# dayoladejo/GADMM

Measured on AMD Instinct MI355X. Metric: wall-clock to 1e-8 objective gap, GADMM linear regression (LinearRegression_Synthetic), lower is better.
Workload: dtype fp64; 1 GPU; model=LinearRegression_Synthetic GADMM closed-form, workers=24, features=50, samples_per_worker=50, global_batch=1200, seq_len=1, parallelism=chain24-over-1gpu

## Files before the change

### csrc/kernels/chain_blocked.hip

```cpp
#include "gadmm_common.h"
#include "gadmm_chain.h"
#include "persist_device.h"
#include "persist_launch.h"
#include <stdlib.h>

namespace {

constexpr int MAXW = 12;
constexpr int HIMG52 = 4 * 64 * 14;
constexpr int EPL = 256;
constexpr long DYN_LDS_BYTES = (long)MAXW * EPL * (16 + 8 + 4);
struct EpochLds {
  int4* sl;
  int2* fl;
  int* st;
};
__device__ __forceinline__ EpochLds epoch_lds(double* base, int v) {
  int4* sl = reinterpret_cast<int4*>(base);
  int2* fl = reinterpret_cast<int2*>(sl + MAXW * EPL);
  int* st = reinterpret_cast<int*>(fl + MAXW * EPL);
  return {sl + v * EPL, fl + v * EPL, st + v * EPL};
}

template <int QT>
__device__ __forceinline__ void quad_load_image(double (&m)[4][QT], const double* img) {
  const int lane = threadIdx.x & 63;
  const double2* p = reinterpret_cast<const double2*>(img) + lane;
#pragma unroll
  for (int t = 0; t < QT; t += 2)
#pragma unroll
    for (int r = 0; r < 4; ++r) {
      const double2 v = p[((t >> 1) * 4 + r) * 64];
      m[r][t] = v.x;
      if (t + 1 < QT) m[r][t + 1] = v.y;
    }
}

template <class PA>
__device__ __forceinline__ void stage_epochs(const PA& a, int q, const EpochLds& el, bool flush) {
  const int lane = threadIdx.x & 63;
  for (int e = lane; e < a.n_epochs; e += 64) {
    el.sl[e] = reinterpret_cast<const int4*>(a.ep_slots)[(long)e * a.n + q];
    if (flush) el.fl[e] = reinterpret_cast<const int2*>(a.ep_flush)[(long)e * a.n + q];
    el.st[e] = a.epoch_start[e];
  }
}
}



template <int QT, bool SYS, bool DYN = false, class PA = PersistArgs>
__device__ __forceinline__ void blocked_objective(const PA& a, double* lds, int v, int lane, int q,
                                                  unsigned long long deadline, __amdgpu_buffer_rsrc_t rob,
                                                  __amdgpu_buffer_rsrc_t rtab, bool local = false) {
  const int d = a.d, n = a.n;
  const long ring_base = 2L * n * 2 * d;
  const EpochLds el = epoch_lds(lds + MAXW * 64 + MAXW * QSTAGE, v);
  int* posl = reinterpret_cast<int*>(el.fl);
  if constexpr (DYN) {
    for (int e = lane; e < a.n_epochs; e += 64) {
      posl[e] = a.ep_pos[(long)e * n + q];
      el.st[e] = a.epoch_start[e];
    }
  }
  const PhaseSlot so = a.slots[DYN ? 0 : q];
  const int li = DYN ? q : so.li, gid = DYN ? q : so.gid;
  int row = DYN ? posl[0] : q;
  const bool in = lane < d;
  double Aq[4][QT];
  quad_load<QT>(Aq, a.A + (long)li * d * d, d, true);
  const double bo = in ? a.b[(long)li * d + lane] : 0.0;
  const double hy = 0.5 * a.yy[li];
  double* xo = lds + v * QSTAGE;
  int ep = 0, next_start = (DYN && a.n_epochs > 1) ? el.st[1] : 0x7fffffff;
  for (int it = a.start_iter;; ++it) {
    if (a.hard_stop > 0 && it > a.hard_stop) return;
    if constexpr (DYN) {
      if (it == next_start) {
        ++ep;
        next_start = ep + 1 < a.n_epochs ? el.st[ep + 1] : 0x7fffffff;
        row = posl[ep];
      }
    }
    const unsigned tag = make_tag(a.epoch, it);
    const long off = (ring_base + ((long)(it % a.ring) * n + row) * d + lane) * 16;
    double x = 0.0;
    for (int spin = 0;; ++spin) {
      const bool ok = !in || load_granule<SYS>(rtab, (int)off, tag, &x);
      if (__all(ok)) break;
      if ((spin & 7) == 7) {
        if (it - a.start_iter >= a.lag) {
          const unsigned long long dv = load_dec<SYS>(&a.decg[(it - a.lag) % a.ring]);
          if ((unsigned)(dv >> 32) == make_tag(a.epoch, it - a.lag) && (unsigned)(dv & 0xffffffffu) != 0u) return;
        }
        if (now_ticks() > deadline) return;
      }
      GADMM_POLL_PAUSE();
    }
    const double qv = quad_gemv<QT>(Aq, in ? x : 0.0, xo);
    const double part = in ? (0.5 * qv - bo) * x : 0.0;
    const double f = wave_sum_f64(part) + hy;
    if (lane == 0) put_granule<SYS>(local, rob, ((it % a.ring) * n + gid) * 16, tag, f);
  }
}

template <int DB, bool SYS, bool TL, bool DYN, bool HALO, bool SWEEP, class PA>
__device__ __forceinline__ void chain_blocked_body(const PA& a) {
  constexpr int QT = DB / 4;
  extern __shared__ __attribute__((aligned(16))) double lds[];
  __shared__ int abort_lds, stop_lds, stop_iter_lds;
  const int d = a.d, n = a.n;
  const int lane = threadIdx.x & 63;
  const int v = __builtin_amdgcn_readfirstlane(threadIdx.x >> 6);
  const int k = a.blk_k, L = a.blk_len, H = 2 * a.blk_k;
  const bool multi = a.nranks > 1;
  const int seg_lo = multi ? a.seg_lo : 0, seg_hi = multi ? a.seg_hi : n - 1;
  const int nseg = seg_hi - seg_lo + 1;
  const int W = (nseg + L - 1) / L;
  const int Wo = (nseg + MAXW - 1) / MAXW;
  const bool dl = SYS && multi && a.blk_dl != 0;
  const unsigned long long deadline = now_ticks() + (unsigned long long)a.timeout_ticks;
  const __amdgpu_buffer_rsrc_t rob = rsrc_of(a.objg);
  const __amdgpu_buffer_rsrc_t rtab = rsrc_of(a.blk_tab);
  const bool packed = SWEEP || (!SYS && a.xcd > 0);
  if (!SWEEP && packed && (blockIdx.x & 7u)) return;
  const int bid = packed ? (int)(blockIdx.x >> 3) : (int)blockIdx.x;
  if (SWEEP && bid > W + Wo) return;
  if (threadIdx.x == 0) {
    abort_lds = 0;
    stop_lds = 0;
  }
  lds_barrier();
  const long ring_base = 2L * n * 2 * d;
  const long etab_base = 2L * n * 2 * d + (long)a.ring * n * d;
  bool local = false;
  if (!SYS && a.xcd > 1) local = xcd_verdict(a.xchk, bid, W + Wo + 1, deadline, &stop_iter_lds, (unsigned)a.xtag);
  if (!SYS && bid == 0 && threadIdx.x == 0) a.ctl->placed = a.xcd > 0 ? (local ? 2 : 1) : 0;

  if (bid == W + Wo) {
    monitor_loop<SYS, GADMM_POLL_SLEEP>(a, lds, rob, deadline, a.start_iter, a.hard_stop,
                                        TL ? a.timeline + (long)bid * a.timeline_iters * 8 : nullptr, 8, v);
    return;
  }

  if (bid >= W) {
    const int q = seg_lo + (bid - W) * MAXW + v;
    if (q <= seg_hi) blocked_objective<QT, SYS, DYN>(a, lds, v, lane, q, deadline, rob, rtab, local);
    return;
  }

  const int g = bid;
  const int s0 = seg_lo + g * L, e0 = min(seg_hi + 1, s0 + L) - 1;
  const int hl = HALO && dl && seg_lo > 0 && (seg_lo % 2) == 1, hr = HALO && dl && seg_hi < n - 1 && (seg_hi % 2) == 1;
  const bool hosted = HALO && dl && (seg_hi - seg_lo + 1 + hl + hr > MAXW);
  const int hd = hosted ? (hr ? 1 : -1) : 0;
  const int hp = hd > 0 ? seg_hi + 1 : (hd < 0 ? seg_lo - 1 : 0);
  const int ra = max(dl ? seg_lo - (hosted ? 0 : hl) : 0, s0 - H), rb = min(dl ? seg_hi + (hosted ? 0 : hr) : n - 1, e0 + H);
  const int nv = rb - ra + 1;
  const int h0 = ra & 1;
  const int u = v < MAXW / 2 ? 2 * v + h0 : 2 * (v - MAXW / 2) + (1 - h0);
  const int p = ra + u;
  const bool active = u < nv;
  const bool owned = active && p >= s0 && p <= e0;
  PhaseSlot sl = DYN ? a.ep_slots[active ? p : 0] : a.slots[active ? p : 0];
  int li = sl.li, w = sl.gid;
  const bool has_l = active && sl.left >= 0, has_r = active && sl.right >= 0;
  const bool head = (p % 2) == 0;
  const int deg = (int)has_l + (int)has_r;
  const double rho = a.rho;
  const bool in = lane < d;
  int vdec = -1;
  for (int u = 0; u < nv && vdec < 0; ++u)
    if (((ra + u) % 2) == 0 && (ra + u < s0 || ra + u > e0)) vdec = u;
  if (vdec < 0 && nv < MAXW) vdec = nv;
  if (vdec < 0) vdec = (ra % 2 == 0) ? 0 : 1;
  const bool dec_wave = u == vdec;

  double* thS = lds;
  double* xs = thS + MAXW * 64;
  double* myx = xs + v * QSTAGE;
  const double* thL = thS + (u > 0 ? u - 1 : u) * 64;
  const double* thR = thS + (u + 1 < nv ? u + 1 : u) * 64;
  const bool nbl = has_l && u > 0, nbr = has_r && u + 1 < nv;
  const int hdir = (hosted && active && p == hp - hd) ? hd : 0;
  const int hq = (hosted && v >= MAXW / 2 && v < MAXW / 2 + 4) ? v - MAXW / 2 : -1;
  const bool rl = dl && has_l && p == ra && hdir != -1, rr = dl && has_r && p == rb && hdir != 1;
  const bool dlh = HALO && dl;
  const bool lb_tail = hl != 0, rb_tail = hr != 0;
  const bool pl = dlh ? (owned && !head && ((p == seg_lo && has_l) || (p == seg_lo + 1 && seg_lo > 0 && !lb_tail)))
                      : rl;
  const bool pr = dlh ? (owned && !head && ((p == seg_hi && has_r) || (p == seg_hi - 1 && seg_hi < n - 1 && !rb_tail)))
                      : rr;
  const bool rpush = dlh ? (pl || pr) : owned && (rl || rr);

  const EpochLds el = epoch_lds(lds + MAXW * 64 + MAXW * QSTAGE, v);
  if constexpr (DYN) {
    stage_epochs(a, active ? p : 0, el, active);
  }
  const int odist = u < s0 - ra ? (s0 - ra) - u : (u > e0 - ra ? u - (e0 - ra) : 0);
  const bool solver = active && odist <= (head ? 2 * k - 1 : 2 * k - 2);
  double Mq[4][QT];
  quad_load<QT>(Mq, a.Minv + ((long)li * a.nvar + a.deg_to_var[deg]) * (long)d * d, d, active);
  auto solve = [&](double r) -> double {
    const double y = quad_gemv<QT>(Mq, in ? r : 0.0, myx);
    return in ? y : 0.0;
  };
  double th = (active && in) ? a.theta[(long)w * d + lane] : 0.0;
  double mu = (active && in) ? a.mu[(long)li * d + lane] : 0.0;
  double bb = (active && in) ? a.b[(long)li * d + lane] : 0.0;
  thS[u * 64 + lane] = th;
  double* Mh = lds + MAXW * 64 + MAXW * QSTAGE;
  double* hst = Mh + HIMG52;
  bool hsl = false, hsr = false;
  if (HALO && hosted) {
    const PhaseSlot sh = a.slots[hp];
    hsl = sh.left >= 0;
    hsr = sh.right >= 0;
    if (hdir != 0) {
      const int deg_h = (int)hsl + (int)hsr;
      quad_store_lds<QT>(Mh, a.Minv + ((long)sh.li * a.nvar + a.deg_to_var[deg_h]) * (long)d * d, d, true);
      hst[lane] = in ? a.theta[(long)sh.gid * d + lane] : 0.0;
      hst[64 + (a.start_iter & 1) * 64 + lane] = in ? a.mu[(long)sh.li * d + lane] : 0.0;
      hst[192 + lane] = in ? a.b[(long)sh.li * d + lane] : 0.0;
    }
  }
  int pending = a.pending_in;
  int ep = 0, next_start = (DYN && a.n_epochs > 1) ? el.st[1] : 0x7fffffff;
  int next_x = a.start_iter + k, xc = 0;
  const int uo_lo = s0 - ra, uo_hi = e0 - ra;
  int blk0 = a.start_iter;
  if (threadIdx.x == 0) stop_iter_lds = 0;
  lds_barrier();

  auto publish = [&](int j) {
    const unsigned tag = make_tag(a.epoch, j + 1);
    const int sel = xc & 1;
    const int base = ((sel * n + p) * 2) * d;
    put_granule<SYS>(local, rtab, (base + lane) * 16, tag, th);
    put_granule<SYS>(local, rtab, (base + d + lane) * 16, tag, mu);
    for (int q = 0; q < a.blk_npeer; ++q)
      if (p >= a.blk_peer_lo[q] && p <= a.blk_peer_hi[q]) {
        const __amdgpu_buffer_rsrc_t rpe = rsrc_of(a.blk_peer_tab[q]);
        store_granule<SYS>(rpe, (base + lane) * 16, tag, th);
        store_granule<SYS>(rpe, (base + d + lane) * 16, tag, mu);
      }
  };
  unsigned long long dv_pref = 0;
  int it = a.start_iter;
  bool hard_stopped = false;
  long long ts[8] = {0, 0, 0, 0, 0, 0, 0, 0};
  const int ring_p = (int)((ring_base + (long)(active ? p : 0) * d + lane) * 16);
  const int ring_slot_bytes = n * d * 16;
  const bool ring_post = owned && in && !(TL && (a.dbg & 2));
  const int ring_l = (int)((ring_base + (long)(rl ? p - 1 : 0) * d + lane) * 16);
  const int ring_r = (int)((ring_base + (long)(rr ? p + 1 : 0) * d + lane) * 16);
  const __amdgpu_buffer_rsrc_t rdl0 = rsrc_of(pl && a.dl_tab[0] ? (const void*)a.dl_tab[0] : (const void*)a.blk_tab);
  const __amdgpu_buffer_rsrc_t rdl1 = rsrc_of(pr && a.dl_tab[1] ? (const void*)a.dl_tab[1] : (const void*)a.blk_tab);
  auto poll_remote = [&](int slot, int j, double& tl, double& tr) -> bool {
    const unsigned tag = make_tag(a.epoch, j);
    const int so = slot * ring_slot_bytes;
    for (int spin = 0;; ++spin) {
      bool g0 = true;
      if (in) {
        if (rl) g0 &= load_granule<SYS>(rtab, ring_l + so, tag, &tl);
        if (rr) g0 &= load_granule<SYS>(rtab, ring_r + so, tag, &tr);
      }
      if (__all(g0)) return true;
      if ((spin & 7) == 7 && now_ticks() > deadline) return false;
      GADMM_POLL_PAUSE();
    }
  };
  auto poll_far = [&](int slot, int j, double& tf) -> bool {
    const unsigned tag = make_tag(a.epoch, j);
    const int so = slot * ring_slot_bytes + (int)((ring_base + (long)(hp + hd) * d + lane) * 16);
    for (int spin = 0;; ++spin) {
      const bool g0 = !in || load_granule<SYS>(rtab, so, tag, &tf);
      if (__all(g0)) return true;
      if ((spin & 7) == 7 && now_ticks() > deadline) return false;
      GADMM_POLL_PAUSE();
    }
  };
  auto push_remote = [&](int slot, int j) {
    const unsigned tag = make_tag(a.epoch, j);
    const int off = ring_p + slot * ring_slot_bytes;
    if (pl) store_granule<SYS>(rdl0, off, tag, th);
    if (pr) store_granule<SYS>(rdl1, off, tag, th);
  };
  bool ring_defer = false;
  int rslot = a.start_iter % a.ring;
  int dslot = (a.start_iter + 1 - a.lag) % a.ring;
  if (dslot < 0) dslot += a.ring;
  for (;; ++it, rslot = rslot + 1 == a.ring ? 0 : rslot + 1, dslot = dslot + 1 == a.ring ? 0 : dslot + 1) {
    if (ring_defer) {
      put_granule<SYS>(local, rtab, ring_p + (rslot == 0 ? a.ring - 1 : rslot - 1) * ring_slot_bytes,
                       make_tag(a.epoch, it - 1), th);
      ring_defer = false;
    }
    if (it > a.max_iter + a.lag) break;
    if (a.hard_stop > 0 && it > a.hard_stop) {
      hard_stopped = true;
      break;
    }
    const bool stamp = TL && v == 0 && it - a.start_iter < a.timeline_iters;
    if (stamp) ts[0] = (long long)now_ticks();
    if constexpr (DYN) {
      if (it == next_start) {
        const unsigned tag = make_tag(a.epoch, it);
        const long eb = etab_base + (long)((ep + 1) & 1) * n * 2 * d;
        if (owned && in) {
          const long base = eb + (long)w * 2 * d;
          put_granule<SYS>(local, rtab, (int)((base + lane) * 16), tag, th);
          put_granule<SYS>(local, rtab, (int)((base + d + lane) * 16), tag, mu);
        }
        ++ep;
        next_start = ep + 1 < a.n_epochs ? el.st[ep + 1] : 0x7fffffff;
        if (active) {
          {
            const int4 s4 = el.sl[ep];
            sl.li = s4.x;
            sl.gid = s4.y;
          }
          const int2 of = el.fl[ep];
          li = sl.li;
          w = sl.gid;
          if (solver) {
            quad_load_image<QT>(Mq, a.minv_pad + ((long)li * a.nvar + a.deg_to_var[deg]) * (long)(512 * ((QT + 1) / 2)));
            bb = in ? a.b[(long)li * d + lane] : 0.0;
          }
          const bool fl = pending && of.x >= 0, fr = pending && of.y >= 0;
          double t0 = 0.0, t1 = 0.0, tl = 0.0, tr = 0.0;
          bool ok = true;
          for (int spin = 0;; ++spin) {
            bool g0 = true;
            if (in) {
              const long b0 = eb + (long)w * 2 * d;
              g0 &= load_granule<SYS>(rtab, (int)((b0 + lane) * 16), tag, &t0);
              g0 &= load_granule<SYS>(rtab, (int)((b0 + d + lane) * 16), tag, &t1);
              if (fl) g0 &= load_granule<SYS>(rtab, (int)((eb + (long)of.x * 2 * d + lane) * 16), tag, &tl);
              if (fr) g0 &= load_granule<SYS>(rtab, (int)((eb + (long)of.y * 2 * d + lane) * 16), tag, &tr);
            }
            if (__all(g0)) break;
            if ((spin & 7) == 7 && now_ticks() > deadline) {
              ok = false;
              break;
            }
            GADMM_POLL_PAUSE();
          }
          if (!ok && lane == 0) abort_lds = 1;
          th = in ? t0 : 0.0;
          double m = in ? t1 : 0.0;
          if (fl) m = m - rho * (tl - th);
          if (fr) m = m + rho * (th - tr);
          mu = in ? m : 0.0;
          thS[u * 64 + lane] = th;
        }
        pending = 0;
        next_x = it + k;
        blk0 = it;
        lds_barrier();
        if (abort_lds) break;
      }
    }
    if (!HALO && it == next_x) {
      if (active && !owned) {
        const unsigned tag = make_tag(a.epoch, it);
        const int sel = xc & 1;
        const int base = ((sel * n + p) * 2) * d;
        double t0 = 0.0, t1 = 0.0;
        bool ok = true;
        for (int spin = 0;; ++spin) {
          bool g0 = true;
          if (in) {
            g0 &= load_granule<SYS>(rtab, (base + lane) * 16, tag, &t0);
            g0 &= load_granule<SYS>(rtab, (base + d + lane) * 16, tag, &t1);
          }
          if (__all(g0)) break;
          if ((spin & 7) == 7 && now_ticks() > deadline) {
            ok = false;
            break;
          }
          GADMM_POLL_PAUSE();
        }
        if (!ok && lane == 0) abort_lds = 1;
        th = in ? t0 : 0.0;
        mu = in ? t1 : 0.0;
        thS[u * 64 + lane] = th;
      }
      lds_barrier();
      if (abort_lds) break;
      blk0 = it;
      next_x = it + k;
      ++xc;
    }
    if (stamp) ts[1] = ts[2] = ts[3] = (long long)now_ticks();

    const int slack = 2 * k - 1 - 2 * (it - blk0);
    if (active && head && u >= uo_lo - slack && u <= uo_hi + slack) {
      double tl = nbl ? thL[lane] : 0.0, tr = nbr ? thR[lane] : 0.0;
      if (rl || rr) {
        if (it == a.start_iter) {
          if (rl && in) tl = a.theta[(long)(p - 1) * d + lane];
          if (rr && in) tr = a.theta[(long)(p + 1) * d + lane];
        } else if (!poll_remote(rslot == 0 ? a.ring - 1 : rslot - 1, it - 1, tl, tr) && lane == 0) {
          abort_lds = 1;
        }
      }
      double m = mu;
      if (pending) {
        if (has_l) m = m - rho * (tl - th);
        if (has_r) m = m + rho * (th - tr);
      }
      mu = m;
      double r = bb - m;
      if (has_l) r = r + rho * tl;
      if (has_r) r = r + rho * tr;
      if (stamp) ts[6] = (long long)now_ticks();
      th = solve(r);
      if (stamp) {
        asm volatile("" ::"v"(th));
        ts[7] = (long long)now_ticks();
      }
      if (rpush && in) push_remote(rslot, it);
      thS[u * 64 + lane] = th;
    }
    if (HALO && hq >= 0) {
      double tf = 0.0;
      if (hd > 0 ? hsr : hsl) {
        if (it == a.start_iter) {
          if (in) tf = a.theta[(long)(hp + hd) * d + lane];
        } else if (!poll_far(rslot == 0 ? a.ring - 1 : rslot - 1, it - 1, tf) && lane == 0) {
          abort_lds = 1;
        }
      }
      const double tn = thS[(hp - hd - ra) * 64 + lane];
      const double tl = hd > 0 ? tn : tf, tr = hd > 0 ? tf : tn;
      const double th_h = hst[lane];
      double m = hst[64 + (it & 1) * 64 + lane];
      if (pending) {
        if (hsl) m = m - rho * (tl - th_h);
        if (hsr) m = m + rho * (th_h - tr);
      }
      if (hq == 0) hst[64 + ((it + 1) & 1) * 64 + lane] = m;
      double r = hst[192 + lane] - m;
      if (hsl) r = r + rho * tl;
      if (hsr) r = r + rho * tr;
      hst[256 + hq * 64 + lane] = quad_rowgroup_lds<QT>(Mh, hq, in ? r : 0.0, myx);
    }
    pending = 1;
    lds_barrier();
    if (stamp) ts[4] = (long long)now_ticks();

    const bool xnext = !HALO && it + 1 == next_x && !(DYN && it + 1 == next_start);
    const bool tstamp = TL && v == MAXW / 2 + ((a.dbg >> 4) & 7) && it - a.start_iter < a.timeline_iters && g < 128;
    long long tt[4] = {0, 0, 0, 0};
    if (active && !head && u >= uo_lo - (slack - 1) && u <= uo_hi + (slack - 1)) {
      if (tstamp) tt[0] = (long long)now_ticks();
      double tl = nbl ? thL[lane] : 0.0, tr = nbr ? thR[lane] : 0.0;
      if (HALO && hdir != 0) {
        double pq[4] = {hst[256 + lane], hst[320 + lane], hst[384 + lane], hst[448 + lane]};
        const double y = quad_reduce(pq);
        const double th_h = in ? y : 0.0;
        hst[lane] = th_h;
        if (hdir > 0) tr = th_h;
        else tl = th_h;
      }
      if ((rl || rr) && !poll_remote(rslot, it, tl, tr) && lane == 0) abort_lds = 1;
      double r = bb - mu;
      if (has_l) r = r + rho * tl;
      if (has_r) r = r + rho * tr;
      if (tstamp) {
        asm volatile("" ::"v"(r));
        tt[1] = (long long)now_ticks();
      }
      const double tn = solve(r);
      if (tstamp) {
        asm volatile("" ::"v"(tn));
        tt[2] = (long long)now_ticks();
      }
      double m = mu;
      if (has_l) m = m - rho * (tl - tn);
      if (has_r) m = m + rho * (tn - tr);
      mu = m;
      th = tn;
      if (rpush && in) push_remote(rslot, it);
      thS[u * 64 + lane] = th;
      if (owned && in && xnext) publish(it);
      ring_defer = ring_post;
      if (a.rres && owned) {
        double rp = 0.0;
        if (in && has_l) rp = fma(tl - tn, tl - tn, rp);
        if (in && has_r) rp = fma(tn - tr, tn - tr, rp);
        const double rs = wave_sum_f64(rp);
        if (lane == 0 && it - 1 < a.max_iter) a.rres[(long)(it - 1) * n + w] = rs;
      }
      if (tstamp) tt[3] = (long long)now_ticks();
    } else if (active && owned && in) {
      if (xnext) publish(it);
      if (ring_post) put_granule<SYS>(local, rtab, ring_p + rslot * ring_slot_bytes, make_tag(a.epoch, it), th);
    }
    if (TL && g < 8 && it - a.start_iter < a.timeline_iters && lane == 0) {
      const long long t_end = (long long)now_ticks();
      a.timeline[((long)(160 + g * MAXW + v) * a.timeline_iters + (it - a.start_iter)) * 8] = t_end;
    }
    if (!(TL && (a.dbg & 1)) && dec_wave && !(active && !head) && lane == 0 && it + 1 - a.start_iter >= a.lag) {
      const int jdec = it + 1 - a.lag;
      const unsigned tj = make_tag(a.epoch, jdec);
      unsigned long long dv = dv_pref;
      if ((unsigned)(dv >> 32) != tj) dv = load_dec<SYS>(&a.decg[dslot]);
      for (int spin = 0; (unsigned)(dv >> 32) != tj; ++spin) {
        if ((spin & 7) == 7 && now_ticks() > deadline) {
          abort_lds = 1;
          break;
        }
        GADMM_POLL_PAUSE();
        dv = load_dec<SYS>(&a.decg[dslot]);
      }
      const unsigned code = (unsigned)(dv & 0xffffffffu);
      if (code && (unsigned)(dv >> 32) == tj) {
        stop_lds = (int)code;
        stop_iter_lds = jdec;
      }
      dv_pref = load_dec<SYS>(&a.decg[dslot + 1 == a.ring ? 0 : dslot + 1]);
    }
    lds_barrier();
    if (tstamp && lane == 0) {
      long long* tl = a.timeline + ((long)(128 + g) * a.timeline_iters + (it - a.start_iter)) * 8;
      for (int q = 0; q < 4; ++q) tl[q] = tt[q];
      tl[4] = (long long)now_ticks();
    }
    if (stamp && lane == 0) {
      long long* tl = a.timeline + ((long)g * a.timeline_iters + (it - a.start_iter)) * 8;
      for (int q = 0; q < 5; ++q) tl[q] = ts[q];
      tl[5] = (long long)now_ticks();
      tl[6] = ts[6];
      tl[7] = ts[7];
    }
    if (abort_lds || stop_lds) {
      ++it;
      break;
    }
  }

  if (ring_defer)
    put_granule<SYS>(local, rtab, ring_p + ((it - 1) % a.ring) * ring_slot_bytes, make_tag(a.epoch, it - 1), th);
  if (owned && in) {
    a.theta[(long)w * d + lane] = th;
    a.mu[(long)li * d + lane] = mu;
  }
  if (threadIdx.x == 0) {
    if (abort_lds) {
      a.ctl->done = 4;
    } else if (g == 0 && stop_lds) {
      a.ctl->done = stop_lds;
      a.ctl->conv_iter = stop_iter_lds;
      a.ctl->iter = it;
      a.ctl->pending = 1;
      a.ctl->monitored = stop_iter_lds;
    } else if (g == 0 && hard_stopped) {
      a.ctl->iter = it;
      a.ctl->pending = 1;
    }
  }
}

typedef __attribute__((address_space(4))) PersistArgs SweepArgs;

template <int DB, bool SYS, bool TL, bool DYN = false, bool HALO = false>
__global__ void __launch_bounds__(64 * MAXW) chain_blocked_kernel(PersistArgs a) {
  chain_blocked_body<DB, SYS, TL, DYN, HALO, false>(a);
}

template <int DB>
__global__ void __launch_bounds__(64 * MAXW) chain_blocked_sweep_kernel(const PersistArgs* __restrict__ batch, int nb) {
  const int j = (int)(blockIdx.x & 7u);
  if (j >= nb) return;
  chain_blocked_body<DB, false, false, false, false, true>(*(const SweepArgs*)(batch + j));
}

template <int DB>
__global__ void __launch_bounds__(64 * MAXW) chain_blocked_dyn_sweep_kernel(const PersistArgs* __restrict__ batch, int nb) {
  const int j = (int)(blockIdx.x & 7u);
  if (j >= nb) return;
  chain_blocked_body<DB, false, false, true, false, true>(*(const SweepArgs*)(batch + j));
}

constexpr int PWW = 8;
constexpr int PCAP = 2 * PWW;

template <int DB, bool SYS>
__global__ void __launch_bounds__(64 * PWW) chain_blocked_pair_kernel(PersistArgs a) {
  constexpr int QT = DB / 4;
  extern __shared__ __attribute__((aligned(16))) double lds[];
  __shared__ int abort_lds, stop_lds, stop_iter_lds;
  const int d = a.d, n = a.n;
  const int lane = threadIdx.x & 63;
  const int v = __builtin_amdgcn_readfirstlane(threadIdx.x >> 6);
  const int k = a.blk_k, L = a.blk_len, H = 2 * a.blk_k;
  const bool multi = a.nranks > 1;
  const int seg_lo = multi ? a.seg_lo : 0, seg_hi = multi ? a.seg_hi : n - 1;
  const int nseg = seg_hi - seg_lo + 1;
  const int W = (nseg + L - 1) / L;
  const int Wo = (nseg + PWW - 1) / PWW;
  const unsigned long long deadline = now_ticks() + (unsigned long long)a.timeout_ticks;
  const __amdgpu_buffer_rsrc_t rob = rsrc_of(a.objg);
  const __amdgpu_buffer_rsrc_t rtab = rsrc_of(a.blk_tab);
  if (threadIdx.x == 0) {
    abort_lds = 0;
    stop_lds = 0;
    stop_iter_lds = 0;
  }
  lds_barrier();
  if ((int)blockIdx.x == W + Wo) {
    monitor_loop<SYS, GADMM_POLL_SLEEP>(a, lds, rob, deadline, a.start_iter, a.hard_stop, nullptr, 0, v);
    return;
  }
  const long ring_base = 2L * n * 2 * d;
  if ((int)blockIdx.x >= W) {
    const int q = seg_lo + ((int)blockIdx.x - W) * PWW + v;
    if (q <= seg_hi) blocked_objective<QT, SYS>(a, lds, v, lane, q, deadline, rob, rtab);
    return;
  }

  const int g = blockIdx.x;
  const int s0 = seg_lo + g * L, e0 = min(seg_hi + 1, s0 + L) - 1;
  const int ra = max(0, s0 - H), rb = min(n - 1, e0 + H);
  const int nv = rb - ra + 1;
  const int uA = 2 * v;
  const bool aHead = ((ra + uA) & 1) == 0;
  const int uH = aHead ? uA : uA + 1, uT = aHead ? uA + 1 : uA;
  const bool actH = uH < nv, actT = uT < nv;
  const int pH = ra + uH, pT = ra + uT;
  const bool ownH = actH && pH >= s0 && pH <= e0, ownT = actT && pT >= s0 && pT <= e0;
  const PhaseSlot slH = a.slots[actH ? pH : 0], slT = a.slots[actT ? pT : 0];
  const bool hlH = actH && slH.left >= 0, hrH = actH && slH.right >= 0;
  const bool hlT = actT && slT.left >= 0, hrT = actT && slT.right >= 0;
  const double rho = a.rho;
  const bool in = lane < d;
  int vdec = 0;
  for (int vv = PWW - 1; vv >= 0; --vv) {
    const int pa = ra + 2 * vv, pb = pa + 1;
    if (2 * vv + 1 < nv && (pa < s0 || pa > e0) && (pb < s0 || pb > e0)) vdec = vv;
  }
  const bool dec_wave = v == vdec;

  double* thS = lds;
  double* bbS = thS + PCAP * 64;
  double* myx = bbS + PCAP * 64 + v * QSTAGE;
  const bool nblH = hlH && uH > 0, nbrH = hrH && uH + 1 < nv;
  const bool nblT = hlT && uT > 0, nbrT = hrT && uT + 1 < nv;

  double MH[3][QT], MT[3][QT], M3[QT];
  quad_load_pair<QT>(MH, MT, M3,
                     a.Minv + ((long)slH.li * a.nvar + a.deg_to_var[(int)hlH + (int)hrH]) * (long)d * d,
                     a.Minv + ((long)slT.li * a.nvar + a.deg_to_var[(int)hlT + (int)hrT]) * (long)d * d, d, actH,
                     actT);
  double thH = (actH && in) ? a.theta[(long)slH.gid * d + lane] : 0.0;
  double muH = (actH && in) ? a.mu[(long)slH.li * d + lane] : 0.0;
  double thT = (actT && in) ? a.theta[(long)slT.gid * d + lane] : 0.0;
  double muT = (actT && in) ? a.mu[(long)slT.li * d + lane] : 0.0;
  if (actH) {
    thS[uH * 64 + lane] = thH;
    bbS[uH * 64 + lane] = in ? a.b[(long)slH.li * d + lane] : 0.0;
  }
  if (actT) {
    thS[uT * 64 + lane] = thT;
    bbS[uT * 64 + lane] = in ? a.b[(long)slT.li * d + lane] : 0.0;
  }
  int pending = a.pending_in;
  lds_barrier();

  auto publish = [&](int j, int p, double th, double mu) {
    const unsigned tag = make_tag(a.epoch, j + 1);
    const int base = (((((j + 1 - a.start_iter) / k) & 1) * n + p) * 2) * d;
    store_granule<SYS>(rtab, (base + lane) * 16, tag, th);
    store_granule<SYS>(rtab, (base + d + lane) * 16, tag, mu);
    for (int q = 0; q < a.blk_npeer; ++q)
      if (p >= a.blk_peer_lo[q] && p <= a.blk_peer_hi[q]) {
        const __amdgpu_buffer_rsrc_t rpe = rsrc_of(a.blk_peer_tab[q]);
        store_granule<SYS>(rpe, (base + lane) * 16, tag, th);
        store_granule<SYS>(rpe, (base + d + lane) * 16, tag, mu);
      }
  };
  unsigned long long dv_pref = 0;
  int it = a.start_iter;
  for (;; ++it) {
    if (it > a.max_iter + a.lag) break;
    if (it > a.start_iter && (it - a.start_iter) % k == 0) {
      const bool needH = actH && !ownH, needT = actT && !ownT;
      if (needH || needT) {
        const unsigned tag = make_tag(a.epoch, it);
        const int bsel = ((it - a.start_iter) / k) & 1;
        const int baseH = ((bsel * n + pH) * 2) * d, baseT = ((bsel * n + pT) * 2) * d;
        double h0 = 0.0, h1 = 0.0, t0 = 0.0, t1 = 0.0;
        bool ok = true;
        for (int spin = 0;; ++spin) {
          bool g0 = true;
          if (in && needH) {
            g0 &= load_granule<SYS>(rtab, (baseH + lane) * 16, tag, &h0);
            g0 &= load_granule<SYS>(rtab, (baseH + d + lane) * 16, tag, &h1);
          }
          if (in && needT) {
            g0 &= load_granule<SYS>(rtab, (baseT + lane) * 16, tag, &t0);
            g0 &= load_granule<SYS>(rtab, (baseT + d + lane) * 16, tag, &t1);
          }
          if (__all(g0)) break;
          if ((spin & 7) == 7 && now_ticks() > deadline) {
            ok = false;
            break;
          }
          GADMM_POLL_PAUSE();
        }
        if (!ok && lane == 0) abort_lds = 1;
        if (needH) {
          thH = in ? h0 : 0.0;
          muH = in ? h1 : 0.0;
          thS[uH * 64 + lane] = thH;
        }
        if (needT) {
          thT = in ? t0 : 0.0;
          muT = in ? t1 : 0.0;
          thS[uT * 64 + lane] = thT;
        }
      }
      lds_barrier();
      if (abort_lds) break;
    }

    if (actH) {
      const double tl = nblH ? thS[(uH - 1) * 64 + lane] : 0.0, tr = nbrH ? thS[(uH + 1) * 64 + lane] : 0.0;
      double m = muH;
      if (pending) {
        if (hlH) m = m - rho * (tl - thH);
        if (hrH) m = m + rho * (thH - tr);
      }
      muH = m;
      double r = bbS[uH * 64 + lane] - m;
      if (hlH) r = r + rho * tl;
      if (hrH) r = r + rho * tr;
      const double y = quad_gemv_pair<QT>(MH, M3, 0, in ? r : 0.0, myx);
      thH = in ? y : 0.0;
      thS[uH * 64 + lane] = thH;
      if (ownH && in)
        store_granule<SYS>(rtab, (int)((ring_base + ((long)(it % a.ring) * n + pH) * d + lane) * 16),
                           make_tag(a.epoch, it), thH);
    }
    pending = 1;
    lds_barrier();

    const bool xnext = (it + 1 - a.start_iter) % k == 0;
    if (actT) {
      const double tl = nblT ? thS[(uT - 1) * 64 + lane] : 0.0, tr = nbrT ? thS[(uT + 1) * 64 + lane] : 0.0;
      double r = bbS[uT * 64 + lane] - muT;
      if (hlT) r = r + rho * tl;
      if (hrT) r = r + rho * tr;
      const double y = quad_gemv_pair<QT>(MT, M3, 1, in ? r : 0.0, myx);
      const double tn = in ? y : 0.0;
      double m = muT;
      if (hlT) m = m - rho * (tl - tn);
      if (hrT) m = m + rho * (tn - tr);
      muT = m;
      thT = tn;
      thS[uT * 64 + lane] = thT;
      if (ownT && in) {
        store_granule<SYS>(rtab, (int)((ring_base + ((long)(it % a.ring) * n + pT) * d + lane) * 16),
                           make_tag(a.epoch, it), thT);
        if (xnext) publish(it, pT, thT, muT);
      }
      if (a.rres && ownT) {
        double rp = 0.0;
        if (in && hlT) rp = fma(tl - tn, tl - tn, rp);
        if (in && hrT) rp = fma(tn - tr, tn - tr, rp);
        const double rs = wave_sum_f64(rp);
        if (lane == 0 && it - 1 < a.max_iter) a.rres[(long)(it - 1) * n + slT.gid] = rs;
      }
    }
    if (ownH && xnext && in) publish(it, pH, thH, muH);
    if (dec_wave && lane == 0 && it + 1 - a.start_iter >= a.lag) {
      const int jdec = it + 1 - a.lag;
      const unsigned tj = make_tag(a.epoch, jdec);
      unsigned long long dvv = dv_pref;
      if ((unsigned)(dvv >> 32) != tj) dvv = load_dec<SYS>(&a.decg[jdec % a.ring]);
      for (int spin = 0; (unsigned)(dvv >> 32) != tj; ++spin) {
        if ((spin & 7) == 7 && now_ticks() > deadline) {
          abort_lds = 1;
          break;
        }
        GADMM_POLL_PAUSE();
        dvv = load_dec<SYS>(&a.decg[jdec % a.ring]);
      }
      const unsigned code = (unsigned)(dvv & 0xffffffffu);
      if (code && (unsigned)(dvv >> 32) == tj) {
        stop_lds = (int)code;
        stop_iter_lds = jdec;
      }
      dv_pref = load_dec<SYS>(&a.decg[(jdec + 1) % a.ring]);
    }
    lds_barrier();
    if (abort_lds || stop_lds) {
      ++it;
      break;
    }
  }

  if (ownH && in) {
    a.theta[(long)slH.gid * d + lane] = thH;
    a.mu[(long)slH.li * d + lane] = muH;
  }
  if (ownT && in) {
    a.theta[(long)slT.gid * d + lane] = thT;
    a.mu[(long)slT.li * d + lane] = muT;
  }
  if (threadIdx.x == 0) {
    if (abort_lds) {
      a.ctl->done = 4;
    } else if (g == 0 && stop_lds) {
      a.ctl->done = stop_lds;
      a.ctl->conv_iter = stop_iter_lds;
      a.ctl->iter = it;
      a.ctl->pending = 1;
      a.ctl->monitored = stop_iter_lds;
    }
  }
}

__global__ void __launch_bounds__(256) pad_image_kernel(const double* __restrict__ M, long mstride,
                                                        const long long* __restrict__ src, long n_el, int batch,
                                                        double* __restrict__ out) {
  const long tot = n_el * batch;
  for (long e = (long)blockIdx.x * 256 + threadIdx.x; e < tot; e += (long)gridDim.x * 256) {
    const long b = e / n_el, k = e - b * n_el;
    const long long s = src[k];
    out[e] = s >= 0 ? M[b * mstride + s] : 0.0;
  }
}

extern "C" {

int gadmm_chain_blocked_plan(int n, int d, int want_k, int* k_out, int* len_out) {
  if (d > 52 || n < 2) return 0;
  int k = want_k > 0 ? want_k : 2;
  int len = MAXW - 4 * k;
  while (len < 1 && k > 1) {
    --k;
    len = MAXW - 4 * k;
  }
  if (len < 1) return 0;
  int cus_xcd = 32;
  const int cus = gadmm_cu_count();
  if (cus >= 8) cus_xcd = cus / 8;
  for (int l = 1; l < len; ++l)
    if ((n + l - 1) / l + (n + MAXW - 1) / MAXW + 1 <= cus_xcd) {
      len = l;
      break;
    }
  if (const char* e = getenv("GADMM_BLOCK_L")) {
    const int want_len = atoi(e);
    if (want_len >= 1 && want_len <= MAXW - 4 * k) len = want_len;
  }
  if (len > n) len = n;
  const int W = (n + len - 1) / len;
  if (W + (n + MAXW - 1) / MAXW + 1 > 256) return 0;
  *k_out = k;
  *len_out = len;
  return W;
}

int gadmm_chain_blocked_plan2(int n, int d, int want_k, int want_pw, int* k_out, int* len_out, int* pw_out) {
  int pw = want_pw;
  if (pw <= 0) {
    const char* e = getenv("GADMM_BLOCK_PW");
    pw = (e && e[0] == '2') ? 2 : 1;
  }
  if (pw == 1) {
    *pw_out = 1;
    return gadmm_chain_blocked_plan(n, d, want_k, k_out, len_out);
  }
  if (d > 52 || n < 2) return 0;
  int k = want_k > 0 ? want_k : 3;
  int len = PCAP - 4 * k;
  while (len < 1 && k > 1) {
    --k;
    len = PCAP - 4 * k;
  }
  if (len < 1) return 0;
  if (const char* e = getenv("GADMM_BLOCK_L")) {
    const int want_len = atoi(e);
    if (want_len >= 1 && want_len < len) len = want_len;
  }
  if (len > n) len = n;
  const int W = (n + len - 1) / len;
  if (W + (n + PWW - 1) / PWW + 1 > 256) return 0;
  *k_out = k;
  *len_out = len;
  *pw_out = 2;
  return W;
}

int gadmm_chain_blocked_pad_dim(int d) { return d <= 32 ? 32 : 52; }
long gadmm_chain_blocked_pad_len(int d) {
  const int qt = gadmm_chain_blocked_pad_dim(d) / 4;
  return 512L * ((qt + 1) / 2);
}
int gadmm_chain_blocked_max_epochs() { return EPL; }

int gadmm_pad_image_f64(const double* M, long mstride, const long long* src, long n_el, int batch, double* out,
                        hipStream_t st) {
  if (!M || !src || !out || n_el < 1 || batch < 1) {
    gadmm_set_error("pad_image: bad arguments");
    return -1;
  }
  const long tot = n_el * batch;
  const int grid = (int)((tot + 255) / 256 < 4096 ? (tot + 255) / 256 : 4096);
  hipLaunchKernelGGL(pad_image_kernel, dim3(grid), dim3(256), 0, st, M, mstride, src, n_el, batch, out);
  GADMM_CHECK(hipGetLastError());
  return 0;
}

int gadmm_chain_blocked_plan_dl(int nseg, int d, int want_k, int* k_out, int* len_out) {
  if (d > 52 || nseg < 1) return 0;
  const char* e = getenv("GADMM_DL_PLAN");
  const bool force_blocked = e && e[0] == 'b' && nseg >= 2;
  if (nseg <= MAXW && !force_blocked) {
    *k_out = 1 << 20;
    *len_out = nseg;
    return 1;
  }
  return gadmm_chain_blocked_plan(nseg, d, want_k, k_out, len_out);
}

long gadmm_chain_blocked_lds(int d, int len) {
  (void)d;
  (void)len;
  return (long)(MAXW * 64 + MAXW * QSTAGE) * 8;
}

long gadmm_chain_blocked_tab_granules(int n, int d, int ring) { return 2L * n * 2 * d + (long)ring * n * d; }
long gadmm_chain_blocked_tab_granules_dyn(int n, int d, int ring) { return 4L * n * 2 * d + (long)ring * n * d; }

int gadmm_chain_blocked_launch(const PersistArgs* args, hipStream_t st) {
  const PersistArgs& a = *args;
  const bool multi = a.nranks > 1;
  const bool dl = a.blk_dl != 0;
  if (dl) {
    const int nseg_dl = a.seg_hi - a.seg_lo + 1;
    const int W_dl = nseg_dl > 0 && a.blk_len > 0 ? (nseg_dl + a.blk_len - 1) / a.blk_len : 0;
    const int nhalo = a.dl_halo ? (int)(a.seg_lo > 0 && a.seg_lo % 2 == 1) + (int)(a.seg_hi < a.n - 1 && a.seg_hi % 2 == 1) : 0;
    const bool hosted_dl = a.dl_halo && nseg_dl + nhalo > MAXW;
    const long span = W_dl == 1 ? (hosted_dl ? nseg_dl : nseg_dl + nhalo) : (long)a.blk_len + 4L * a.blk_k;
    if (hosted_dl && (nhalo != 1 || nseg_dl < 8)) {
      gadmm_set_error("blocked chain kernel (data-local halo): a hosted halo needs one hosted side and >= 4 tails");
      return -1;
    }
    if (!multi || !a.sys_scope || a.blk_pw != 1 || a.n_epochs != 0 || a.blk_npeer != 0 || a.blk_k < 1 ||
        a.blk_len < 1 || nseg_dl < 1 || span > MAXW || (W_dl > 1 && a.ring < 2 * a.blk_k + 4) ||
        (a.seg_lo > 0 && !a.dl_tab[0]) || (a.seg_hi < a.n - 1 && !a.dl_tab[1]) ||
        (a.dl_halo && (W_dl != 1 || nseg_dl < 2 || a.d > 52))) {
      gadmm_set_error("blocked chain kernel (data-local): unsupported configuration (seg %d..%d, L=%d, k=%d)",
                      a.seg_lo, a.seg_hi, a.blk_len, a.blk_k);
      return -1;
    }
  }
  if (a.blk_k < 1 || a.blk_len < 1 || (!dl && a.blk_len + 4 * a.blk_k > (a.blk_pw == 2 ? PCAP : MAXW)) || a.d > 52 ||
      !a.blk_tab || !a.dec_push ||
      (!multi && (!a.has_monitor || a.n != a.n_local)) ||
      (multi && (a.seg_lo < 0 || a.seg_hi < a.seg_lo || a.seg_hi >= a.n || a.blk_npeer < 0 || a.blk_npeer > 8 ||
                 (a.blk_npeer > 0 && !a.blk_peer_tab) || a.start_iter != 1 || a.pending_in != 0 || !a.sys_scope))) {
    gadmm_set_error("blocked chain kernel: unsupported configuration");
    return -1;
  }
  if (a.lag < 1) {
    gadmm_set_error("blocked chain kernel: lag must be at least 1");
    return -1;
  }
  PersistArgs ka = a;
  void* kargs[] = {&ka};
  const int nseg = multi ? a.seg_hi - a.seg_lo + 1 : a.n;
  const int W = (nseg + a.blk_len - 1) / a.blk_len;
  if (a.blk_pw == 2 && a.n_epochs == 0) {
    if (a.blk_len + 4 * a.blk_k > PCAP || a.timeline) {
      gadmm_set_error("blocked chain kernel (pw=2): L + 4k > %d or timeline requested", PCAP);
      return -1;
    }
    const int Wo2 = (nseg + PWW - 1) / PWW;
    const int blocks2 = W + Wo2 + (a.has_monitor ? 1 : 0);
    long lds2 = (long)(2 * PCAP * 64 + PWW * QSTAGE) * 8;
    if (lds2 < (long)a.n * 8) lds2 = (long)a.n * 8;
    const void* fn2 = a.sys_scope ? (a.d <= 32 ? (const void*)chain_blocked_pair_kernel<32, true>
                                               : (const void*)chain_blocked_pair_kernel<52, true>)
                                  : (a.d <= 32 ? (const void*)chain_blocked_pair_kernel<32, false>
                                               : (const void*)chain_blocked_pair_kernel<52, false>);
    return gadmm_persist_launch({fn2, 64 * PWW, (size_t)lds2, blocks2, "blocked chain kernel", false}, &ka, kargs, st);
  }
  const int Wo = (nseg + MAXW - 1) / MAXW;
  const int blocks = W + Wo + (a.has_monitor ? 1 : 0);
  long lds = gadmm_chain_blocked_lds(a.d, a.blk_len);
  if (lds < (long)a.n * 8) lds = (long)a.n * 8;
  if (lds > 160 * 1024) {
    gadmm_set_error("blocked chain kernel: %ld B of LDS", lds);
    return -1;
  }
  const void* fn;
  const bool tl = a.timeline != nullptr;
  if (a.n_epochs > 0) {
    if (multi || tl || a.sys_scope || !a.epoch_start || !a.ep_slots || !a.ep_pos || !a.minv_pad || !a.ep_flush ||
        a.hard_stop < 0 || (a.hard_stop > 0 && a.hard_stop < a.start_iter) || a.n_epochs > EPL) {
      gadmm_set_error("blocked chain kernel: dynamic epochs need one GPU, epoch tables (at most %d epochs per "
                      "launch), the padded inverse image (gadmm_chain_blocked_pad_len), no timeline", EPL);
      return -1;
    }
    lds = gadmm_chain_blocked_lds(a.d, a.blk_len) + DYN_LDS_BYTES;
    fn = a.d <= 32 ? (const void*)chain_blocked_kernel<32, false, false, true>
                   : (const void*)chain_blocked_kernel<52, false, false, true>;
  } else if (a.sys_scope && dl && a.dl_halo) {
    if (tl) {
      gadmm_set_error("blocked chain kernel: no timeline build of the data-local halo mode");
      return -1;
    }
    fn = a.d <= 32 ? (const void*)chain_blocked_kernel<32, true, false, false, true>
                   : (const void*)chain_blocked_kernel<52, true, false, false, true>;
    lds += (long)(HIMG52 + 512) * 8;
  } else if (a.sys_scope) {
    if (tl) fn = a.d <= 32 ? (const void*)chain_blocked_kernel<32, true, true> : (const void*)chain_blocked_kernel<52, true, true>;
    else fn = a.d <= 32 ? (const void*)chain_blocked_kernel<32, true, false> : (const void*)chain_blocked_kernel<52, true, false>;
  } else {
    if (tl) fn = a.d <= 32 ? (const void*)chain_blocked_kernel<32, false, true> : (const void*)chain_blocked_kernel<52, false, true>;
    else fn = a.d <= 32 ? (const void*)chain_blocked_kernel<32, false, false> : (const void*)chain_blocked_kernel<52, false, false>;
  }
  {
    const char* e = getenv("GADMM_BLK_DBG");
    ka.dbg = e ? atoi(e) : 0;
  }
  return gadmm_persist_launch({fn, 64 * MAXW, (size_t)lds, blocks, "blocked chain kernel", true}, &ka, kargs, st);
}

int gadmm_chain_blocked_sweep_capacity() { return 8; }

int gadmm_chain_blocked_sweep_launch(const PersistArgs* batch, int nb, PersistArgs* host_stage, PersistArgs* dev_stage,
                                     hipStream_t st) {
  if (nb < 1 || nb > gadmm_chain_blocked_sweep_capacity()) {
    gadmm_set_error("blocked sweep: %d solves, one launch takes 1..%d", nb, gadmm_chain_blocked_sweep_capacity());
    return -1;
  }
  if (!batch || !host_stage || !dev_stage) {
    gadmm_set_error("blocked sweep: null batch or staging buffer");
    return -1;
  }
  int blocks[8], max_blocks = 0, sum_blocks = 0;
  long lds = gadmm_chain_blocked_lds(0, 0);
  for (int j = 1; j < nb; ++j)
    if ((batch[j].d <= 32) != (batch[0].d <= 32)) {
      gadmm_set_error("blocked sweep: solves of different register classes (d = %d and %d; d <= 32 or 33..52)",
                      batch[0].d, batch[j].d);
      return -1;
    }
  for (int j = 0; j < nb; ++j) {
    const PersistArgs& a = batch[j];
    if (a.nranks > 1 || a.sys_scope || a.n_epochs > 0 || a.blk_pw == 2 || a.timeline || a.blk_dl || a.dl_halo ||
        a.blk_npeer != 0 || a.hard_stop != 0 || a.cont) {
      gadmm_set_error("blocked sweep: solve %d is multi-rank, system-scope, dynamic, paired-wave, instrumented or "
                      "data-local (one-GPU static 12-wave solves only)", j);
      return -1;
    }
    if (!a.xchk) {
      gadmm_set_error("blocked sweep: solve %d has no placement-check buffer (xchk)", j);
      return -1;
    }
    if (a.blk_k < 1 || a.blk_len < 1 || a.blk_len + 4 * a.blk_k > MAXW || a.d < 1 || a.d > 52 || a.n < 2 ||
        !a.blk_tab || !a.dec_push || !a.objg || !a.decg || !a.ctl || !a.trace || !a.theta || !a.mu || !a.slots ||
        !a.Minv || !a.A || !a.b || !a.yy || !a.has_monitor || a.n != a.n_local) {
      gadmm_set_error("blocked sweep: solve %d: unsupported configuration", j);
      return -1;
    }
    if (a.lag < 1 || a.ring <= a.lag + 1 || a.start_iter + a.max_iter + a.lag >= (1 << 20)) {
      gadmm_set_error("blocked sweep: solve %d: ring/lag/tag range", j);
      return -1;
    }
    for (int i = 0; i < j; ++i) {
      const PersistArgs& o = batch[i];
      if (o.ctl == a.ctl || o.trace == a.trace || o.theta == a.theta || o.mu == a.mu || o.blk_tab == a.blk_tab ||
          o.objg == a.objg || o.decg == a.decg || o.xchk == a.xchk || (a.tstamp && o.tstamp == a.tstamp)) {
        gadmm_set_error("blocked sweep: solves %d and %d share a buffer that both write", i, j);
        return -1;
      }
    }
    const int W = (a.n + a.blk_len - 1) / a.blk_len, Wo = (a.n + MAXW - 1) / MAXW;
    blocks[j] = W + Wo + 1;
    if (blocks[j] > XCHK) {
      gadmm_set_error("blocked sweep: solve %d has %d workgroups, the placement check holds %d", j, blocks[j], XCHK);
      return -1;
    }
    sum_blocks += blocks[j];
    if (blocks[j] > max_blocks) max_blocks = blocks[j];
    if (lds < (long)a.n * 8) lds = (long)a.n * 8;
  }
  if (lds > 160 * 1024) {
    gadmm_set_error("blocked sweep: %ld B of LDS", lds);
    return -1;
  }
  const void* fn = batch[0].d <= 32 ? (const void*)chain_blocked_sweep_kernel<32> : (const void*)chain_blocked_sweep_kernel<52>;
  const long cap = gadmm_resident_capacity(fn, 64 * MAXW, (size_t)lds);
  const long cus_xcd = gadmm_cu_count() / 8;
  if (sum_blocks > cap) {
    gadmm_set_error("blocked sweep: %d workgroups but only %ld can be resident", sum_blocks, cap);
    return -2;
  }
  for (int j = 0; j < nb; ++j)
    if (blocks[j] > cus_xcd) {
      gadmm_set_error("blocked sweep: solve %d has %d workgroups but an XCD has %ld CUs", j, blocks[j], cus_xcd);
      return -2;
    }
  if (lds > 65536) GADMM_CHECK(hipFuncSetAttribute(fn, hipFuncAttributeMaxDynamicSharedMemorySize, (int)lds));
  int dbg = 0, xenv = -1;
  if (const char* e = getenv("GADMM_BLK_DBG")) dbg = atoi(e);
  if (const char* e = getenv("GADMM_XCD")) xenv = atoi(e);
  for (int j = 0; j < nb; ++j) {
    PersistArgs& ka = host_stage[j];
    ka = batch[j];
    ka.dbg = dbg;
    const int x = xenv >= 0 ? xenv : ka.xcd;
    ka.xcd = x >= 2 ? 2 : 1;
    ka.xtag = (int)gadmm_next_xtag();
  }
  GADMM_CHECK(hipMemcpyAsync(dev_stage, host_stage, (size_t)nb * sizeof(PersistArgs), hipMemcpyHostToDevice, st));
  const PersistArgs* dbatch = dev_stage;
  void* kargs[] = {&dbatch, &nb};
  GADMM_CHECK(hipLaunchKernel(fn, dim3(8 * max_blocks), dim3(64 * MAXW), kargs, (size_t)lds, st));
  GADMM_CHECK(hipGetLastError());
  return 0;
}

int gadmm_chain_blocked_dyn_sweep_launch(const PersistArgs* batch, int nb, PersistArgs* host_stage,
                                         PersistArgs* dev_stage, hipStream_t st) {
  if (nb < 1 || nb > gadmm_chain_blocked_sweep_capacity()) {
    gadmm_set_error("blocked dynamic sweep: %d solves, one launch takes 1..%d", nb, gadmm_chain_blocked_sweep_capacity());
    return -1;
  }
  if (!batch || !host_stage || !dev_stage) {
    gadmm_set_error("blocked dynamic sweep: null batch or staging buffer");
    return -1;
  }
  int blocks[8], max_blocks = 0, sum_blocks = 0;
  long lds = gadmm_chain_blocked_lds(0, 0) + DYN_LDS_BYTES;
  for (int j = 1; j < nb; ++j)
    if ((batch[j].d <= 32) != (batch[0].d <= 32)) {
      gadmm_set_error("blocked dynamic sweep: solves of different register classes (d = %d and %d; d <= 32 or "
                      "33..52)", batch[0].d, batch[j].d);
      return -1;
    }
  for (int j = 0; j < nb; ++j) {
    const PersistArgs& a = batch[j];
    if (a.n_epochs < 1) {
      gadmm_set_error("blocked dynamic sweep: solve %d is static (no epochs): it belongs in the static sweep", j);
      return -1;
    }
    if (a.nranks > 1 || a.sys_scope || a.blk_pw == 2 || a.timeline || a.blk_dl || a.dl_halo || a.blk_npeer != 0) {
      gadmm_set_error("blocked dynamic sweep: solve %d is multi-rank, system-scope, paired-wave, instrumented or "
                      "data-local (one-GPU 12-wave solves only)", j);
      return -1;
    }
    if (a.n_epochs > EPL) {
      gadmm_set_error("blocked dynamic sweep: solve %d has %d epochs, a launch stages at most %d", j, a.n_epochs, EPL);
      return -1;
    }
    if (!a.epoch_start || !a.ep_slots || !a.ep_pos || !a.ep_flush || !a.minv_pad) {
      gadmm_set_error("blocked dynamic sweep: solve %d lacks epoch tables or the padded inverse image "
                      "(gadmm_chain_blocked_pad_len)", j);
      return -1;
    }
    if (a.hard_stop < 0 || (a.hard_stop > 0 && a.hard_stop < a.start_iter)) {
      gadmm_set_error("blocked dynamic sweep: solve %d: hard stop %d before its start %d", j, a.hard_stop, a.start_iter);
      return -1;
    }
    if (!a.xchk) {
      gadmm_set_error("blocked dynamic sweep: solve %d has no placement-check buffer (xchk)", j);
      return -1;
    }
    if (a.blk_k < 1 || a.blk_len < 1 || a.blk_len + 4 * a.blk_k > MAXW || a.d < 1 || a.d > 52 || a.n < 2 ||
        !a.blk_tab || !a.dec_push || !a.objg || !a.decg || !a.ctl || !a.trace || !a.theta || !a.mu || !a.slots ||
        !a.Minv || !a.A || !a.b || !a.yy || !a.has_monitor || a.n != a.n_local) {
      gadmm_set_error("blocked dynamic sweep: solve %d: unsupported configuration", j);
      return -1;
    }
    if (a.lag < 1 || a.ring <= a.lag + 1 || a.start_iter + a.max_iter + a.lag >= (1 << 20)) {
      gadmm_set_error("blocked dynamic sweep: solve %d: ring/lag/tag range", j);
      return -1;
    }
    for (int i = 0; i < j; ++i) {
      const PersistArgs& o = batch[i];
      if (o.ctl == a.ctl || o.trace == a.trace || o.theta == a.theta || o.mu == a.mu || o.blk_tab == a.blk_tab ||
          o.objg == a.objg || o.decg == a.decg || o.xchk == a.xchk || (a.tstamp && o.tstamp == a.tstamp) ||
          (a.rres && o.rres == a.rres)) {
        gadmm_set_error("blocked dynamic sweep: solves %d and %d share a buffer that both write", i, j);
        return -1;
      }
    }
    const int W = (a.n + a.blk_len - 1) / a.blk_len, Wo = (a.n + MAXW - 1) / MAXW;
    blocks[j] = W + Wo + 1;
    if (blocks[j] > XCHK) {
      gadmm_set_error("blocked dynamic sweep: solve %d has %d workgroups, the placement check holds %d", j, blocks[j],
                      XCHK);
      return -1;
    }
    sum_blocks += blocks[j];
    if (blocks[j] > max_blocks) max_blocks = blocks[j];
    if (lds < (long)a.n * 8) lds = (long)a.n * 8;
  }
  if (lds > 160 * 1024) {
    gadmm_set_error("blocked dynamic sweep: %ld B of LDS", lds);
    return -1;
  }
  const void* fn = batch[0].d <= 32 ? (const void*)chain_blocked_dyn_sweep_kernel<32>
                                    : (const void*)chain_blocked_dyn_sweep_kernel<52>;
  const long cap = gadmm_resident_capacity(fn, 64 * MAXW, (size_t)lds);
  const long cus_xcd = gadmm_cu_count() / 8;
  if (sum_blocks > cap) {
    gadmm_set_error("blocked dynamic sweep: %d workgroups but only %ld can be resident", sum_blocks, cap);
    return -2;
  }
  for (int j = 0; j < nb; ++j)
    if (blocks[j] > cus_xcd) {
      gadmm_set_error("blocked dynamic sweep: solve %d has %d workgroups but an XCD has %ld CUs", j, blocks[j], cus_xcd);
      return -2;
    }
  if (lds > 65536) GADMM_CHECK(hipFuncSetAttribute(fn, hipFuncAttributeMaxDynamicSharedMemorySize, (int)lds));
  int dbg = 0, xenv = -1;
  if (const char* e = getenv("GADMM_BLK_DBG")) dbg = atoi(e);
  if (const char* e = getenv("GADMM_XCD")) xenv = atoi(e);
  for (int j = 0; j < nb; ++j) {
    PersistArgs& ka = host_stage[j];
    ka = batch[j];
    ka.dbg = dbg;
    const int x = xenv >= 0 ? xenv : ka.xcd;
    ka.xcd = x >= 2 ? 2 : 1;
    ka.xtag = (int)gadmm_next_xtag();
  }
  GADMM_CHECK(hipMemcpyAsync(dev_stage, host_stage, (size_t)nb * sizeof(PersistArgs), hipMemcpyHostToDevice, st));
  const PersistArgs* dbatch = dev_stage;
  void* kargs[] = {&dbatch, &nb};
  GADMM_CHECK(hipLaunchKernel(fn, dim3(8 * max_blocks), dim3(64 * MAXW), kargs, (size_t)lds, st));
  GADMM_CHECK(hipGetLastError());
  return 0;
}

}
```

Before: 1.712 ms.

## Move decision polling before first barrier and snapshot stop flags per wave

Moves the convergence-decision poll earlier in the iteration, before the head-phase barrier, and picks the polling wave more carefully: it avoids head waves and halo helper waves and prefers inactive or non-owned ones. For the non-SYS path, stop and abort flags are snapshotted into scalar registers after the first barrier, so the loop-exit check does not reread LDS after the second barrier. The abort checks after epoch and exchange barriers are dropped for the non-SYS path. This aims to take the decision poll off the critical path of the tail-phase solve and to shorten LDS traffic around the barriers. The trade-off is that stop is observed with slightly different timing and aborts are detected later.

```diff
diff --git a/csrc/kernels/chain_blocked.hip b/csrc/kernels/chain_blocked.hip
--- a/csrc/kernels/chain_blocked.hip
+++ b/csrc/kernels/chain_blocked.hip
@@ -169,12 +169,19 @@
   const int deg = (int)has_l + (int)has_r;
   const double rho = a.rho;
   const bool in = lane < d;
-  int vdec = -1;
-  for (int u = 0; u < nv && vdec < 0; ++u)
-    if (((ra + u) % 2) == 0 && (ra + u < s0 || ra + u > e0)) vdec = u;
-  if (vdec < 0 && nv < MAXW) vdec = nv;
-  if (vdec < 0) vdec = (ra % 2 == 0) ? 0 : 1;
-  const bool dec_wave = u == vdec;
+  int vdec = -1, cdec = 3;
+  for (int vv = 0; vv < MAXW; ++vv) {
+    const int uu = vv < MAXW / 2 ? 2 * vv + h0 : 2 * (vv - MAXW / 2) + (1 - h0);
+    const bool act = uu < nv, hd_ = act && ((ra + uu) % 2) == 0;
+    const bool own = act && ra + uu >= s0 && ra + uu <= e0;
+    if (hd_ || (hosted && vv >= MAXW / 2 && vv < MAXW / 2 + 4)) continue;
+    const int c = act ? (own ? 2 : 0) : 1;
+    if (c < cdec) {
+      cdec = c;
+      vdec = vv;
+    }
+  }
+  const bool dec_wave = v == vdec;
 
   double* thS = lds;
   double* xs = thS + MAXW * 64;
@@ -290,6 +297,28 @@
   int rslot = a.start_iter % a.ring;
   int dslot = (a.start_iter + 1 - a.lag) % a.ring;
   if (dslot < 0) dslot += a.ring;
+  auto poll_decision = [&]() {
+    if (!(TL && (a.dbg & 1)) && dec_wave && lane == 0 && it + 1 - a.start_iter >= a.lag) {
+      const int jdec = it + 1 - a.lag;
+      const unsigned tj = make_tag(a.epoch, jdec);
+      unsigned long long dv = dv_pref;
+      if ((unsigned)(dv >> 32) != tj) dv = load_dec<SYS>(&a.decg[dslot]);
+      for (int spin = 0; (unsigned)(dv >> 32) != tj; ++spin) {
+        if ((spin & 7) == 7 && now_ticks() > deadline) {
+          abort_lds = 1;
+          break;
+        }
+        GADMM_POLL_PAUSE();
+        dv = load_dec<SYS>(&a.decg[dslot]);
+      }
+      const unsigned code = (unsigned)(dv & 0xffffffffu);
+      if (code && (unsigned)(dv >> 32) == tj) {
+        stop_lds = (int)code;
+        stop_iter_lds = jdec;
+      }
+      dv_pref = load_dec<SYS>(&a.decg[dslot + 1 == a.ring ? 0 : dslot + 1]);
+    }
+  };
   for (;; ++it, rslot = rslot + 1 == a.ring ? 0 : rslot + 1, dslot = dslot + 1 == a.ring ? 0 : dslot + 1) {
     if (ring_defer) {
       put_granule<SYS>(local, rtab, ring_p + (rslot == 0 ? a.ring - 1 : rslot - 1) * ring_slot_bytes,
@@ -325,7 +354,9 @@
           w = sl.gid;
           if (solver) {
             quad_load_image<QT>(Mq, a.minv_pad + ((long)li * a.nvar + a.deg_to_var[deg]) * (long)(512 * ((QT + 1) / 2)));
-            bb = in ? a.b[(long)li * d + lane] : 0.0;
+            int bl = lane;
+            asm volatile("" : "+v"(bl));
+            bb = in ? a.b[(long)li * d + bl] : 0.0;
           }
           const bool fl = pending && of.x >= 0, fr = pending && of.y >= 0;
           double t0 = 0.0, t1 = 0.0, tl = 0.0, tr = 0.0;
@@ -358,7 +389,8 @@
         next_x = it + k;
         blk0 = it;
         lds_barrier();
-        if (abort_lds) break;
+        if constexpr (SYS)
+          if (abort_lds) break;
       }
     }
     if (!HALO && it == next_x) {
@@ -387,7 +419,8 @@
         thS[u * 64 + lane] = th;
       }
       lds_barrier();
-      if (abort_lds) break;
+      if constexpr (SYS)
+        if (abort_lds) break;
       blk0 = it;
       next_x = it + k;
       ++xc;
@@ -446,16 +479,25 @@
       if (hsr) r = r + rho * tr;
       hst[256 + hq * 64 + lane] = quad_rowgroup_lds<QT>(Mh, hq, in ? r : 0.0, myx);
     }
+    poll_decision();
     pending = 1;
     lds_barrier();
+    int stop_v = 0, abort_v = 0;
+    if constexpr (!SYS) {
+      stop_v = stop_lds;
+      abort_v = abort_lds;
+      asm volatile("" ::: "memory");
+    }
     if (stamp) ts[4] = (long long)now_ticks();
 
     const bool xnext = !HALO && it + 1 == next_x && !(DYN && it + 1 == next_start);
     const bool tstamp = TL && v == MAXW / 2 + ((a.dbg >> 4) & 7) && it - a.start_iter < a.timeline_iters && g < 128;
     long long tt[4] = {0, 0, 0, 0};
+    int flags_s;
     if (active && !head && u >= uo_lo - (slack - 1) && u <= uo_hi + (slack - 1)) {
       if (tstamp) tt[0] = (long long)now_ticks();
       double tl = nbl ? thL[lane] : 0.0, tr = nbr ? thR[lane] : 0.0;
+      flags_s = __builtin_amdgcn_readfirstlane(stop_v) | __builtin_amdgcn_readfirstlane(abort_v);
       if (HALO && hdir != 0) {
         double pq[4] = {hst[256 + lane], hst[320 + lane], hst[384 + lane], hst[448 + lane]};
         const double y = quad_reduce(pq);
@@ -494,33 +536,16 @@
         if (lane == 0 && it - 1 < a.max_iter) a.rres[(long)(it - 1) * n + w] = rs;
       }
       if (tstamp) tt[3] = (long long)now_ticks();
-    } else if (active && owned && in) {
-      if (xnext) publish(it);
-      if (ring_post) put_granule<SYS>(local, rtab, ring_p + rslot * ring_slot_bytes, make_tag(a.epoch, it), th);
+    } else {
+      flags_s = __builtin_amdgcn_readfirstlane(stop_v) | __builtin_amdgcn_readfirstlane(abort_v);
+      if (active && owned && in) {
+        if (xnext) publish(it);
+        if (ring_post) put_granule<SYS>(local, rtab, ring_p + rslot * ring_slot_bytes, make_tag(a.epoch, it), th);
+      }
     }
     if (TL && g < 8 && it - a.start_iter < a.timeline_iters && lane == 0) {
       const long long t_end = (long long)now_ticks();
       a.timeline[((long)(160 + g * MAXW + v) * a.timeline_iters + (it - a.start_iter)) * 8] = t_end;
-    }
-    if (!(TL && (a.dbg & 1)) && dec_wave && !(active && !head) && lane == 0 && it + 1 - a.start_iter >= a.lag) {
-      const int jdec = it + 1 - a.lag;
-      const unsigned tj = make_tag(a.epoch, jdec);
-      unsigned long long dv = dv_pref;
-      if ((unsigned)(dv >> 32) != tj) dv = load_dec<SYS>(&a.decg[dslot]);
-      for (int spin = 0; (unsigned)(dv >> 32) != tj; ++spin) {
-        if ((spin & 7) == 7 && now_ticks() > deadline) {
-          abort_lds = 1;
-          break;
-        }
-        GADMM_POLL_PAUSE();
-        dv = load_dec<SYS>(&a.decg[dslot]);
-      }
-      const unsigned code = (unsigned)(dv & 0xffffffffu);
-      if (code && (unsigned)(dv >> 32) == tj) {
-        stop_lds = (int)code;
-        stop_iter_lds = jdec;
-      }
-      dv_pref = load_dec<SYS>(&a.decg[dslot + 1 == a.ring ? 0 : dslot + 1]);
     }
     lds_barrier();
     if (tstamp && lane == 0) {
@@ -535,7 +560,8 @@
       tl[6] = ts[6];
       tl[7] = ts[7];
     }
-    if (abort_lds || stop_lds) {
+    if constexpr (SYS) flags_s = abort_lds | stop_lds;
+    if (flags_s) {
       ++it;
       break;
     }
```

Measured after the change: 1.617 ms (median of 6 runs). -5.5%, faster.
